# lbcb-sci/raven

Hardware: AMD Instinct MI355X
Metric: read Gbase/s through overlap+polish (higher is better)
Workload: dtype u32

## Files before the change

### raven_amd/csrc/map.hip

```cpp
#include <algorithm>

#include <cstring>

#include "engine.h"
#include "wave.h"
#ifdef RVN_TEST_HOOKS
#include "../../include/raven_hip_test.h"
#include "abi.h"
#endif

namespace rvn {

namespace {

template <typename V>
__device__ __forceinline__ bool index_find(const V* __restrict__ u_val, const u32* __restrict__ u_start,
                                           const u32* __restrict__ table, int shift, V v, u32* start, u32* count) {
  const u32 b = static_cast<u32>(static_cast<u64>(v) >> shift);
  u32 lo = table[b], hi = table[b + 1];
  const u32 end = hi;
  while (lo < hi) {
    const u32 mid = lo + ((hi - lo) >> 1);
    if (u_val[mid] < v) lo = mid + 1;
    else hi = mid;
  }
  if (lo < end && u_val[lo] == v) {
    *start = u_start[lo];
    *count = u_start[lo + 1] - *start;
    return true;
  }
  return false;
}

template <typename V>
__global__ void match_count_kernel(const V* __restrict__ q_val, const u64* __restrict__ q_org, u64 nq,
                                   const V* __restrict__ u_val, const u32* __restrict__ u_start,
                                   const u32* __restrict__ table, int shift, u32 n_keys,
                                   const u64* __restrict__ s_org, u32 occurrence, int avoid_equal,
                                   int avoid_symmetric, u32* __restrict__ q_start, u32* __restrict__ q_n,
                                   u32* __restrict__ q_cnt, u8* __restrict__ filtered, const u64* __restrict__ direct) {
  u64 q = static_cast<u64>(blockIdx.x) * blockDim.x + threadIdx.x;
  if (q >= nq) return;
  const V v = q_val[q];
  const u32 qid = origin_id(q_org[q]);
  u32 start = 0, count = 0, cnt = 0;
  u8 filt = 0;
  bool found;
  if (direct) {
    const u64 ent = direct[static_cast<u64>(v)];
    count = static_cast<u32>(ent >> 32);
    found = count != 0;
    start = found ? static_cast<u32>(ent) : 0u;
  } else {
    found = n_keys && index_find<V>(u_val, u_start, table, shift, v, &start, &count);
  }
  if (found) {
    if (count > occurrence) {
      filt = 1;
      count = 0;
    } else {
      for (u32 j = 0; j < count; ++j) {
        const u32 rid = origin_id(s_org[start + j]);
        if (avoid_equal && qid == rid) continue;
        if (avoid_symmetric && qid > rid) continue;
        ++cnt;
      }
    }
  }
  q_start[q] = start;
  q_n[q] = count;
  q_cnt[q] = cnt;
  if (filtered) filtered[q] = filt;
}

__global__ void match_emit_kernel(const u64* __restrict__ q_org, u64 nq, const u64* __restrict__ s_org,
                                  const u32* __restrict__ q_start, const u32* __restrict__ q_n,
                                  const u64* __restrict__ m_off, int avoid_equal, int avoid_symmetric,
                                  u64* __restrict__ m_grp, u64* __restrict__ m_pos) {
  u64 q = static_cast<u64>(blockIdx.x) * blockDim.x + threadIdx.x;
  if (q >= nq) return;
  const u32 count = q_n[q];
  if (count == 0) return;
  const u64 qo = q_org[q];
  const u32 qid = origin_id(qo);
  const u64 lhs_pos = static_cast<u32>(qo) >> 1;
  const u32 qstrand = static_cast<u32>(qo) & 1u;
  const u32 start = q_start[q];
  u64 o = m_off[q];
  for (u32 j = 0; j < count; ++j) {
    const u64 ro = s_org[start + j];
    const u32 rid = origin_id(ro);
    if (avoid_equal && qid == rid) continue;
    if (avoid_symmetric && qid > rid) continue;
    const u64 rhs_pos = static_cast<u32>(ro) >> 1;
    const u64 strand = (qstrand == (static_cast<u32>(ro) & 1u)) ? 1 : 0;
    const u64 diagonal = !strand ? rhs_pos + lhs_pos : rhs_pos - lhs_pos + (3ULL << 30);
    m_grp[o] = (((static_cast<u64>(rid) << 1) | strand) << 32) | diagonal;
    m_pos[o] = (lhs_pos << 32) | rhs_pos;
    ++o;
  }
}

template <bool EMIT>
__global__ __launch_bounds__(256) void join_kernel(const u32* __restrict__ u_start, u32 n_runs,
                                                  const u64* __restrict__ s_org, u32 occurrence, int all_query,
                                                  int avoid_equal, int avoid_symmetric, u32 first, u32 q_lo, u32 q_hi,
                                                  u32* __restrict__ read_cnt, const u64* __restrict__ seg_off,
                                                  u32* __restrict__ cursor, u64* __restrict__ m_grp,
                                                  u64* __restrict__ m_pos) {
  const u32 run = blockIdx.x * blockDim.x + threadIdx.x;
  if (run >= n_runs) return;
  const u32 s = u_start[run];
  const u32 c = u_start[run + 1] - s;
  const u32 f = run_foreign_prefix(s_org, s, c);
  if (c - f > occurrence || c == f) return;
  if (c == 1 && avoid_equal) return;
  for (u32 i = 0; i < c; ++i) {
    const u64 qo = s_org[s + i];
    if (!all_query && !(qo & kQueryFlag)) continue;
    const u32 qid = origin_id(qo);
    if (qid < q_lo || qid >= q_hi) continue;
    u32 cnt = 0;
    for (u32 j = f; j < c; ++j) {
      const u32 rid = origin_id(s_org[s + j]);
      if (avoid_equal && qid == rid) continue;
      if (avoid_symmetric && qid > rid) continue;
      ++cnt;
    }
    if (cnt == 0) continue;
    if (!EMIT) {
      atomicAdd(&read_cnt[qid - first], cnt);
    } else {
      u64 o = seg_off[qid - first] + atomicAdd(&cursor[qid - first], cnt);
      const u64 lhs_pos = static_cast<u32>(qo) >> 1;
      const u32 qstrand = static_cast<u32>(qo) & 1u;
      for (u32 j = f; j < c; ++j) {
        const u64 ro = s_org[s + j];
        const u32 rid = origin_id(ro);
        if (avoid_equal && qid == rid) continue;
        if (avoid_symmetric && qid > rid) continue;
        const u64 rhs_pos = static_cast<u32>(ro) >> 1;
        const u64 strand = (qstrand == (static_cast<u32>(ro) & 1u)) ? 1 : 0;
        const u64 diagonal = !strand ? rhs_pos + lhs_pos : rhs_pos - lhs_pos + (3ULL << 30);
        m_grp[o] = (((static_cast<u64>(rid) << 1) | strand) << 32) | diagonal;
        m_pos[o] = (lhs_pos << 32) | rhs_pos;
        ++o;
      }
    }
  }
}

__global__ void gather_u64_by_u32_kernel(const u64* __restrict__ src, const u32* __restrict__ idx,
                                         u64* __restrict__ dst, u32 n) {
  u32 i = blockIdx.x * blockDim.x + threadIdx.x;
  if (i < n) dst[i] = src[idx[i]];
}

template <bool PAY>
__device__ void wave_sort_segment(u64* __restrict__ k0, u64* __restrict__ k1, u64* __restrict__ p0,
                                  u64* __restrict__ p1, u64 b, u64 n, u32* hist) {
  const int lane = lane_id();
  const unsigned long long lt = lanemask_lt();
  u32* h_cur = hist;
  u32* h_nxt = hist + 256;
  for (int i = lane; i < 256; i += 64) h_nxt[i] = 0;
  __builtin_amdgcn_wave_barrier();
  u64 o = 0, a = ~0ULL;
  for (u64 i = lane; i < n; i += 64) {
    const u64 key = k0[b + i];
    o |= key;
    a &= key;
    atomicAdd(&h_nxt[key & 0xFF], 1u);
  }
#pragma unroll
  for (int off = 32; off > 0; off >>= 1) {
    o |= __shfl_xor(o, off, 64);
    a &= __shfl_xor(a, off, 64);
  }
  const u64 varying = o ^ a;
  int cur = 0;
  bool have_counts = true;
  int counted_shift = 0;
  for (int shift = 0; shift < 64; shift += 8) {
    if (((varying >> shift) & 0xFF) == 0) continue;
    const u64* kin = cur ? k1 : k0;
    const u64* pin = cur ? p1 : p0;
    u64* kout = cur ? k0 : k1;
    u64* pout = cur ? p0 : p1;
    __builtin_amdgcn_wave_barrier();
    if (have_counts && counted_shift == shift) {
      u32* t = h_cur;
      h_cur = h_nxt;
      h_nxt = t;
    } else {
      for (int i = lane; i < 256; i += 64) h_cur[i] = 0;
      __builtin_amdgcn_wave_barrier();
      for (u64 i = lane; i < n; i += 64) atomicAdd(&h_cur[(kin[b + i] >> shift) & 0xFF], 1u);
    }
    int nshift = shift + 8;
    while (nshift < 64 && ((varying >> nshift) & 0xFF) == 0) nshift += 8;
    have_counts = nshift < 64;
    counted_shift = nshift;
    __builtin_amdgcn_wave_barrier();
    {
      const u32 h0 = h_cur[4 * lane], h1 = h_cur[4 * lane + 1], h2 = h_cur[4 * lane + 2], h3 = h_cur[4 * lane + 3];
      const u32 s = h0 + h1 + h2 + h3;
      const u32 ex = wave_inclusive_sum(s) - s;
      __builtin_amdgcn_wave_barrier();
      h_cur[4 * lane] = ex;
      h_cur[4 * lane + 1] = ex + h0;
      h_cur[4 * lane + 2] = ex + h0 + h1;
      h_cur[4 * lane + 3] = ex + h0 + h1 + h2;
      for (int i = lane; i < 256; i += 64) h_nxt[i] = 0;
    }
    __builtin_amdgcn_wave_barrier();
    for (u64 base = 0; base < n; base += 256) {
      u64 key[4], pay[4];
      bool valid[4];
#pragma unroll
      for (int x = 0; x < 4; ++x) {
        const u64 i = base + 64 * x + lane;
        valid[x] = i < n;
        key[x] = 0;
        pay[x] = 0;
        if (valid[x]) {
          key[x] = kin[b + i];
          if (PAY) pay[x] = pin[b + i];
        }
      }
#pragma unroll
      for (int x = 0; x < 4; ++x) {
        if (base + 64 * x >= n) break;
        const unsigned d = static_cast<unsigned>((key[x] >> shift) & 0xFF);
        const unsigned long long peers = match_digit8(d, valid[x]);
        u32 before = 0;
        if (valid[x]) before = h_cur[d];
        __builtin_amdgcn_wave_barrier();
        const u32 rank = before + __popcll(peers & lt);
        if (valid[x] && (peers & lt) == 0) h_cur[d] = before + __popcll(peers);
        __builtin_amdgcn_wave_barrier();
        if (valid[x]) {
          kout[b + rank] = key[x];
          if (PAY) pout[b + rank] = pay[x];
          if (have_counts) atomicAdd(&h_nxt[(key[x] >> nshift) & 0xFF], 1u);
        }
      }
    }
    __threadfence_block();
    cur ^= 1;
  }
  if (cur) {
    for (u64 i = lane; i < n; i += 64) {
      k0[b + i] = k1[b + i];
      if (PAY) p0[b + i] = p1[b + i];
    }
    __threadfence_block();
  }
}

template <int NT, bool PAY>
constexpr size_t seg_sort_lds_bytes(u32 cap) {
  return static_cast<size_t>(cap) * 8 * (PAY ? 4 : 2) + (NT / 64) * 256 * 2 + 32 + (NT / 64) * 16;
}
template <int NT, bool PAY>
__device__ void block_sort_lds(u64* __restrict__ keys, u64* __restrict__ pays, u64 b, u32 n, u32 cap, unsigned char* smem) {
  constexpr int NW = NT / 64;
  static_assert(NT == 64 || NT == 256, "one wave or four");
  u64* s_k = reinterpret_cast<u64*>(smem);
  u64* s_p = s_k + 2 * static_cast<size_t>(cap);
  u16* wave_cnt = reinterpret_cast<u16*>(s_p + (PAY ? 2 * static_cast<size_t>(cap) : 0));
  u32* s4 = reinterpret_cast<u32*>(wave_cnt + NW * 256);
  u64* s_or = reinterpret_cast<u64*>(s4 + 8);
  u64* s_and = s_or + NW;
  const int lane = lane_id();
  const int w = threadIdx.x >> 6;
  u64 o = 0, a = ~0ULL;
  for (u32 i = threadIdx.x; i < n; i += NT) {
    const u64 k = keys[b + i];
    s_k[i] = k;
    if (PAY) s_p[i] = pays[b + i];
    o |= k;
    a &= k;
  }
#pragma unroll
  for (int x = 32; x > 0; x >>= 1) {
    o |= __shfl_xor(o, x, 64);
    a &= __shfl_xor(a, x, 64);
  }
  if (lane == 0) {
    s_or[w] = o;
    s_and[w] = a;
  }
  __syncthreads();
  u64 all_or = 0, all_and = ~0ULL;
#pragma unroll
  for (int x = 0; x < NW; ++x) {
    all_or |= s_or[x];
    all_and &= s_and[x];
  }
  const u64 varying = all_or ^ all_and;
  const u32 per = (n + NW - 1) / NW;
  const u32 q0 = min(n, w * per), q1 = min(n, q0 + per);
  const unsigned long long lt = lanemask_lt();
  u32 cur = 0;
  for (int shift = 0; shift < 64; shift += 8) {
    if (((varying >> shift) & 0xFF) == 0) continue;
    const u64* kin = s_k + static_cast<size_t>(cur) * cap;
    u64* kout = s_k + static_cast<size_t>(cur ^ 1) * cap;
    const u64* pin = s_p + static_cast<size_t>(cur) * cap;
    u64* pout = s_p + static_cast<size_t>(cur ^ 1) * cap;
    for (int i = threadIdx.x; i < NW * 256; i += NT) wave_cnt[i] = 0;
    __syncthreads();
    u16* my_cnt = wave_cnt + w * 256;
    for (u32 base = q0; base < q1; base += 64) {
      const u32 i = base + lane;
      const bool valid = i < q1;
      const unsigned d = valid ? static_cast<unsigned>((kin[i] >> shift) & 0xFF) : 0;
      const unsigned long long peers = match_digit8(d, valid);
      if (valid && (peers & lt) == 0) my_cnt[d] += static_cast<u16>(__popcll(peers));
      __builtin_amdgcn_wave_barrier();
    }
    __syncthreads();
    if (NT == 256) {
      const int t = threadIdx.x;
      u32 c[NW], tot = 0;
#pragma unroll
      for (int x = 0; x < NW; ++x) {
        c[x] = wave_cnt[x * 256 + t];
        tot += c[x];
      }
      u32 total;
      u32 run = block_exclusive_sum_256<u32>(tot, s4, &total);
#pragma unroll
      for (int x = 0; x < NW; ++x) {
        wave_cnt[x * 256 + t] = static_cast<u16>(run);
        run += c[x];
      }
    } else {
      const u32 h0 = wave_cnt[4 * lane], h1 = wave_cnt[4 * lane + 1], h2 = wave_cnt[4 * lane + 2], h3 = wave_cnt[4 * lane + 3];
      const u32 sum = h0 + h1 + h2 + h3;
      const u32 ex = wave_inclusive_sum(sum) - sum;
      __builtin_amdgcn_wave_barrier();
      wave_cnt[4 * lane] = static_cast<u16>(ex);
      wave_cnt[4 * lane + 1] = static_cast<u16>(ex + h0);
      wave_cnt[4 * lane + 2] = static_cast<u16>(ex + h0 + h1);
      wave_cnt[4 * lane + 3] = static_cast<u16>(ex + h0 + h1 + h2);
    }
    __syncthreads();
    for (u32 base = q0; base < q1; base += 64) {
      const u32 i = base + lane;
      const bool valid = i < q1;
      u64 k = 0, pv = 0;
      if (valid) {
        k = kin[i];
        if (PAY) pv = pin[i];
      }
      const unsigned d = static_cast<unsigned>((k >> shift) & 0xFF);
      const unsigned long long peers = match_digit8(d, valid);
      u32 before = 0;
      if (valid) before = my_cnt[d];
      __builtin_amdgcn_wave_barrier();
      if (valid && (peers & lt) == 0) my_cnt[d] = static_cast<u16>(before + __popcll(peers));
      __builtin_amdgcn_wave_barrier();
      if (valid) {
        const u32 dst = before + __popcll(peers & lt);
        kout[dst] = k;
        if (PAY) pout[dst] = pv;
      }
    }
    __syncthreads();
    cur ^= 1;
  }
  const u64* kfin = s_k + static_cast<size_t>(cur) * cap;
  const u64* pfin = s_p + static_cast<size_t>(cur) * cap;
  for (u32 i = threadIdx.x; i < n; i += NT) {
    keys[b + i] = kfin[i];
    if (PAY) pays[b + i] = pfin[i];
  }
}

constexpr int kSegClasses = 5;
__constant__ u32 kSegClassCap[kSegClasses] = {256, 512, 1024, 2048, 4096};
static const u32 kSegClassCapHost[kSegClasses] = {256, 512, 1024, 2048, 4096};
__global__ __launch_bounds__(256) void seg_class_list_kernel(const u64* __restrict__ off, u32 n_seg, u32* __restrict__ lists,
                                                            u32* __restrict__ cnt) {
  const u32 t = blockIdx.x * blockDim.x + threadIdx.x;
  int cls = -1;
  if (t < n_seg) {
    const u64 n = off[t + 1] - off[t];
    if (n >= 2) {
      cls = kSegClasses;
      for (int c = kSegClasses - 1; c >= 0; --c)
        if (n <= kSegClassCap[c]) cls = c;
    }
  }
  const int lane = lane_id();
  for (int c = 0; c <= kSegClasses; ++c) {
    const unsigned long long m = __ballot(cls == c);
    if (!m) continue;
    u32 base = 0;
    if (lane == 0) base = atomicAdd(cnt + c, static_cast<u32>(__popcll(m)));
    base = __shfl(base, 0, 64);
// ... 461 lines not shown
    const u32 nblk = (n + 63) >> 6;
    for (u32 b2 = lane; b2 < nblk; b2 += 64) maskbuf[b2] = 0;
    u32 j = tail_idx[longest];
    chain_sync<GLOBAL>();
    u32 left = longest;
    for (int b2 = static_cast<int>(j >> 6); b2 >= 0 && left; --b2) {
      const u32 idx = (static_cast<u32>(b2) << 6) + static_cast<u32>(lane);
      const u32 pr = idx < n ? static_cast<u32>(pred[idx]) : 0u;
      const unsigned long long cont = __ballot(lane > 0 && idx < n && pr + 1 == idx);
      unsigned long long m = 0;
      while (left && static_cast<int>(j >> 6) == b2) {
        const u32 l = j & 63u;
        const unsigned long long upto = l == 63 ? ~0ULL : ((2ULL << l) - 1ULL);
        const unsigned long long stops = ~cont & upto;
        u32 r = 63u - static_cast<u32>(__builtin_clzll(stops));
        if (l - r + 1 > left) r = l + 1 - left;
        m |= upto & ~((1ULL << r) - 1ULL);
        left -= l - r + 1;
        j = static_cast<u32>(__shfl(static_cast<int>(pr), static_cast<int>(r), 64));
      }
      if (lane == 0) maskbuf[b2] = m;
    }
    chain_sync<GLOBAL>();
    u32 at = 0;
    for (u32 b2 = 0; b2 < nblk; ++b2) {
      const unsigned long long m = maskbuf[b2];
      if ((m >> lane) & 1ULL) tail_idx[at + static_cast<u32>(__popcll(m & ((1ULL << lane) - 1ULL)))] = static_cast<IdxT>((b2 << 6) + lane);
      at += static_cast<u32>(__popcll(m));
    }
    chain_sync<GLOBAL>();
    for (u32 m = lane; m < longest; m += 64) tail_pos[m] = p[tail_idx[m]];
    chain_sync<GLOBAL>();
  }
  chain_emit_wave([&](u32 m) { return tail_pos[m]; }, longest, strand, g0, lhs_id, k, chain, min_matches, gap, slots,
                  slot_flags, anchors, anchor_base, slot_aoff, slot_acnt);
}

constexpr int kChainClasses = 8;
__constant__ u32 kChainClassCap[kChainClasses] = {128, 256, 512, 768, 1024, 2048, 4096, kChainBigCap};
static const u32 kChainClassCapHost[kChainClasses] = {128, 256, 512, 768, 1024, 2048, 4096, kChainBigCap};
inline size_t chain_class_lds(u32 cap) {
  return static_cast<size_t>(cap + 1) * 8 + (cap / 64 + 2) * 8 + static_cast<size_t>(cap + 2) * 2 + static_cast<size_t>(cap) * 2 + 64;
}

__global__ __launch_bounds__(64) void chain_kernel(const u64* __restrict__ grp, const u64* __restrict__ pos,
                                                  const u64* __restrict__ iv_begin, const u64* __restrict__ iv_end,
                                                  const u32* __restrict__ iv_read, const u32* __restrict__ list,
                                                  u32 n_list, u32 cap, const u32* __restrict__ ids, u32 first, u32 k,
                                                  u32 chain, u32 min_matches, u32 gap, u32 slot_div,
                                                  u64* __restrict__ g_tail_pos, u32* __restrict__ g_tail_idx,
                                                  u32* __restrict__ g_pred, u64* __restrict__ g_mask,
                                                  Overlap* __restrict__ slots, u8* __restrict__ slot_flags,
                                                  u64* __restrict__ anchors, u64* __restrict__ slot_aoff,
                                                  u32* __restrict__ slot_acnt) {
  extern __shared__ __attribute__((aligned(16))) unsigned char chain_smem[];
  if (blockIdx.x >= n_list) return;
  const u32 t = list[blockIdx.x];
  const u64 b = iv_begin[t];
  const u32 n = static_cast<u32>(iv_end[t] - b);
  const u64 g0 = grp[b];
  const bool strand = (g0 >> 32) & 1;
  const u32 lhs_id = ids[first + iv_read[t]];
  const u64 slot_base = (b + slot_div - 1) / slot_div;
  if (cap) {
    u64* tail_pos = reinterpret_cast<u64*>(chain_smem);
    u64* maskbuf = tail_pos + (cap + 1);
    u16* tail_idx = reinterpret_cast<u16*>(maskbuf + (cap / 64 + 2));
    u16* pred = tail_idx + (cap + 2);
    chain_wave<u16, false>(pos + b, n, strand, g0, lhs_id, k, chain, min_matches, gap, tail_pos, tail_idx, pred, maskbuf,
                           slots + slot_base, slot_flags + slot_base, anchors ? anchors + b : nullptr, b,
                           slot_aoff ? slot_aoff + slot_base : nullptr, slot_acnt ? slot_acnt + slot_base : nullptr);
  } else {
    chain_wave<u32, true>(pos + b, n, strand, g0, lhs_id, k, chain, min_matches, gap, g_tail_pos + b + t,
                          g_tail_idx + b + t, g_pred + b, g_mask + (b >> 6) + t, slots + slot_base,
                          slot_flags + slot_base, anchors ? anchors + b : nullptr, b,
                          slot_aoff ? slot_aoff + slot_base : nullptr, slot_acnt ? slot_acnt + slot_base : nullptr);
  }
}

__global__ __launch_bounds__(256) void chain_class_list_kernel(const u64* __restrict__ iv_begin,
                                                              const u64* __restrict__ iv_end, u32 n_iv, u32 chain,
                                                              u32* __restrict__ lists, u32* __restrict__ cnt) {
  const u32 t = blockIdx.x * blockDim.x + threadIdx.x;
  int cls = -1;
  if (t < n_iv) {
    const u64 n = iv_end[t] - iv_begin[t];
    if (n > kChainSmallCap && n >= chain) {
      cls = kChainClasses;
      for (int c = kChainClasses - 1; c >= 0; --c)
        if (n <= kChainClassCap[c]) cls = c;
    }
  }
  const int lane = lane_id();
  for (int c = 0; c <= kChainClasses; ++c) {
    const unsigned long long m = __ballot(cls == c);
    if (!m) continue;
    u32 base = 0;
    if (lane == 0) base = atomicAdd(cnt + c, static_cast<u32>(__popcll(m)));
    base = __shfl(base, 0, 64);
    if (cls == c) lists[static_cast<size_t>(c) * n_iv + base + __popcll(m & ((1ULL << lane) - 1ULL))] = t;
  }
}

__global__ void compact_overlaps_kernel(const Overlap* __restrict__ slots, const u8* __restrict__ flags,
                                        const u32* __restrict__ scan, u64 n_slots, Overlap* __restrict__ out) {
  u64 i = static_cast<u64>(blockIdx.x) * blockDim.x + threadIdx.x;
  if (i < n_slots && flags[i]) out[scan[i]] = slots[i];
}

__global__ void compact_aux_kernel(const u64* __restrict__ slot_aoff, const u32* __restrict__ slot_acnt,
                                   const u8* __restrict__ flags, const u32* __restrict__ scan, u64 n_slots,
                                   u64* __restrict__ aoff, u32* __restrict__ acnt) {
  u64 i = static_cast<u64>(blockIdx.x) * blockDim.x + threadIdx.x;
  if (i < n_slots && flags[i]) {
    aoff[scan[i]] = slot_aoff[i];
    acnt[scan[i]] = slot_acnt[i];
  }
}

__global__ void read_ovl_off_kernel(const u64* __restrict__ seg_off, const u32* __restrict__ scan, u32 slot_div,
                                    u32 n, u32* __restrict__ out) {
  u32 i = blockIdx.x * blockDim.x + threadIdx.x;
  if (i < n) out[i] = scan[(seg_off[i] + slot_div - 1) / slot_div];
}

}

void chain_matches(Engine& e, const ReadsDev& r, u32 first, u32 last, u64 H, MapOut& out) {
  hipStream_t s = e.stream;
  const u32 nr = last - first;
  u32* ovl_read_off = out.ovl_read_off.get<u32>(static_cast<size_t>(nr) + 1);
  u64* seg_off = e.map.seg_off.as<u64>();
  if (H == 0) {
    RVN_HIP(hipMemsetAsync(ovl_read_off, 0, (static_cast<size_t>(nr) + 1) * 4, s));
    return;
  }
  u64* g0 = e.map.m_grp[0].as<u64>();
  u64* g1 = e.map.m_grp[1].as<u64>();
  u64* p0 = e.map.m_pos[0].as<u64>();
  u64* p1 = e.map.m_pos[1].as<u64>();
  {
    StageTimer t(e, StageTimes::kSegSort);
    u32* lists = e.map.chain_big.get<u32>(static_cast<size_t>(nr) * (kSegClasses + 1) + 16);
    u32* d_cnt = lists + static_cast<size_t>(nr) * (kSegClasses + 1);
    RVN_HIP(hipMemsetAsync(d_cnt, 0, (kSegClasses + 1) * 4, s));
    seg_class_list_kernel<<<div_up(nr, 256), 256, 0, s>>>(seg_off, nr, lists, d_cnt);
    RVN_LAUNCH_CHECK();
    read_back(e, d_cnt, (kSegClasses + 1) * 4);
    u32 n_cls[kSegClasses + 1];
    std::memcpy(n_cls, e.h_pin, sizeof(n_cls));
    static bool attr_set = false;
    if (!attr_set) {
      RVN_HIP(hipFuncSetAttribute(reinterpret_cast<const void*>(seg_sort_group_lds_kernel<256>),
                                  hipFuncAttributeMaxDynamicSharedMemorySize,
                                  static_cast<int>(seg_sort_lds_bytes<256, true>(kSegClassCapHost[kSegClasses - 1]))));
      attr_set = true;
    }
    if (n_cls[kSegClasses])
      RVN_KLAUNCH(kKSegSortGroup, seg_sort_group_big_kernel<<<div_up(n_cls[kSegClasses], 4), 256, 0, s>>>(
                                      g0, g1, p0, p1, seg_off, lists + static_cast<size_t>(kSegClasses) * nr, n_cls[kSegClasses]));
    for (int c = kSegClasses - 1; c >= 0; --c) {
      if (!n_cls[c]) continue;
      const u32 cap = kSegClassCapHost[c];
      const u32* list = lists + static_cast<size_t>(c) * nr;
      if (cap <= 512)
        RVN_KLAUNCH(kKSegSortGroup, seg_sort_group_lds_kernel<64><<<n_cls[c], 64, seg_sort_lds_bytes<64, true>(cap), s>>>(
                                        g0, p0, seg_off, list, n_cls[c], cap));
      else
        RVN_KLAUNCH(kKSegSortGroup, seg_sort_group_lds_kernel<256><<<n_cls[c], 256, seg_sort_lds_bytes<256, true>(cap), s>>>(
                                        g0, p0, seg_off, list, n_cls[c], cap));
    }
    t.stop();
  }
  u32 NI = 0;
  const u64 n_slots4 = (H + 3) / 4 + 1;
  {
    StageTimer t(e, StageTimes::kIntervals);
    u64* slot_begin = e.map.iv_slot_begin.get<u64>(n_slots4 + 1);
    u64* slot_end = e.map.iv_slot_end.get<u64>(n_slots4 + 1);
    u32* iv_cnt = e.map.iv_cnt.get<u32>(static_cast<size_t>(nr) + 1);
    u32* iv_off = e.map.iv_off.get<u32>(static_cast<size_t>(nr) + 2);
    RVN_KLAUNCH(kKIntervals, intervals_kernel<<<div_up(nr, 4), 256, 0, s>>>(g0, seg_off, nr, e.bandwidth, slot_begin, slot_end, iv_cnt));
    exclusive_scan_u32_u32(iv_cnt, iv_off, nr, e.scratch.scan_tmp, s);
    NI = static_cast<u32>(read_back(e, iv_off + nr, 4));
    out.n_intervals = NI;
    if (NI) {
      u64* iv_begin = e.map.iv_begin.get<u64>(static_cast<size_t>(NI) + 1);
      u64* iv_end = e.map.iv_end.get<u64>(static_cast<size_t>(NI) + 1);
      u32* iv_read = e.scratch.tmp_b.get<u32>(static_cast<size_t>(NI) + 1);
      RVN_KLAUNCH(kKIntervalsGather, intervals_gather_kernel<<<div_up(nr, 4), 256, 0, s>>>(
                                         slot_begin, slot_end, seg_off, iv_off, nr, iv_begin, iv_end, iv_read));
    }
    t.stop();
  }
  if (NI == 0) {
    RVN_HIP(hipMemsetAsync(ovl_read_off, 0, (static_cast<size_t>(nr) + 1) * 4, s));
    return;
  }
  const u32 slot_div = std::max(1u, std::min(4u, e.chain));
  const u64 n_slots = (H + slot_div - 1) / slot_div + 1;
  Overlap* slots = e.map.ovl_slots.get<Overlap>(n_slots + 1);
  u8* slot_flags = e.map.ovl_flags.get<u8>(n_slots + 1);
  {
    StageTimer t(e, StageTimes::kChain);
    u64* iv_begin = e.map.iv_begin.as<u64>();
    u64* iv_end = e.map.iv_end.as<u64>();
    u32* iv_read = e.scratch.tmp_b.as<u32>();
    u32* lists = e.map.chain_big.get<u32>(static_cast<size_t>(NI) * (kChainClasses + 1) + 16);
    u32* d_cnt = lists + static_cast<size_t>(NI) * (kChainClasses + 1);
    RVN_HIP(hipMemsetAsync(d_cnt, 0, (kChainClasses + 1) * 4, s));
    chain_class_list_kernel<<<div_up(NI, 256), 256, 0, s>>>(iv_begin, iv_end, NI, e.chain, lists, d_cnt);
    RVN_LAUNCH_CHECK();
    read_back(e, d_cnt, (kChainClasses + 1) * 4);
    u32 n_cls[kChainClasses + 1];
    std::memcpy(n_cls, e.h_pin, sizeof(n_cls));
    static bool attr_set = false;
    if (!attr_set) {
      RVN_HIP(hipFuncSetAttribute(reinterpret_cast<const void*>(chain_kernel), hipFuncAttributeMaxDynamicSharedMemorySize,
                                  static_cast<int>(chain_class_lds(kChainBigCap))));
      RVN_HIP(hipFuncSetAttribute(reinterpret_cast<const void*>(seg_sort_pos_lds_kernel<256>),
                                  hipFuncAttributeMaxDynamicSharedMemorySize,
                                  static_cast<int>(seg_sort_lds_bytes<256, false>(kChainBigCap))));
      attr_set = true;
    }
    if (n_cls[kChainClasses])
      RVN_KLAUNCH(kKSegSortPos, seg_sort_pos_big_kernel<<<div_up(n_cls[kChainClasses], 4), 256, 0, s>>>(
                                    p0, p1, iv_begin, iv_end, lists + static_cast<size_t>(kChainClasses) * NI, n_cls[kChainClasses]));
    for (int c = kChainClasses - 1; c >= 0; --c) {
      if (!n_cls[c]) continue;
      const u32 cap = kChainClassCapHost[c];
      const u32* list = lists + static_cast<size_t>(c) * NI;
      if (cap <= 512)
        RVN_KLAUNCH(kKSegSortPos, seg_sort_pos_lds_kernel<64><<<n_cls[c], 64, seg_sort_lds_bytes<64, false>(cap), s>>>(
                                      p0, iv_begin, iv_end, list, n_cls[c], cap));
      else
        RVN_KLAUNCH(kKSegSortPos, seg_sort_pos_lds_kernel<256><<<n_cls[c], 256, seg_sort_lds_bytes<256, false>(cap), s>>>(
                                      p0, iv_begin, iv_end, list, n_cls[c], cap));
    }
    u32* lis_min = e.map.lis_min.get<u32>(H + NI + 1);
    u32* lis_pred = e.map.lis_pred.get<u32>(H + 1);
    u64* lis_tail = e.map.lis_tail.get<u64>(H + NI + 1);
    u64* lis_mask = e.map.lis_mask.get<u64>((H >> 6) + NI + 2);
    RVN_HIP(hipMemsetAsync(slot_flags, 0, n_slots + 1, s));
    u64* anchors = nullptr;
    u64* slot_aoff = nullptr;
    u32* slot_acnt = nullptr;
    if (e.map.keep_anchors) {
      anchors = out.anchors.get<u64>(H + 1);
      slot_aoff = e.map.anc_slot_off.get<u64>(n_slots + 1);
      slot_acnt = e.map.anc_slot_cnt.get<u32>(n_slots + 1);
    }
    RVN_KLAUNCH(kKChainSmall, chain_small_kernel<<<div_up(NI, 64), 64, 0, s>>>(
                                  g0, p0, iv_begin, iv_end, iv_read, NI, r.id.as<u32>(), first, e.k, e.chain, e.matches,
                                  e.gap, slot_div, slots, slot_flags, anchors, slot_aoff, slot_acnt));
    {
      for (int c = kChainClasses; c >= 0; --c) {
        if (!n_cls[c]) continue;
        const u32 cap = c < kChainClasses ? kChainClassCapHost[c] : 0u;
        const size_t lds = cap ? chain_class_lds(cap) : 0;
        RVN_KLAUNCH(kKChain, chain_kernel<<<n_cls[c], 64, lds, s>>>(g0, p0, iv_begin, iv_end, iv_read,
                                                                   lists + static_cast<size_t>(c) * NI, n_cls[c], cap,
                                                                   r.id.as<u32>(), first, e.k, e.chain, e.matches, e.gap,
                                                                   slot_div, lis_tail, lis_min, lis_pred, lis_mask, slots,
                                                                   slot_flags, anchors, slot_aoff, slot_acnt));
      }
    }
    t.stop();
  }
  {
    StageTimer t(e, StageTimes::kCompact);
    u32* scan = e.map.ovl_scan.get<u32>(n_slots + 2);
    exclusive_scan_u8_u32(slot_flags, scan, n_slots, e.scratch.scan_tmp, s);
    const u32 O = static_cast<u32>(read_back(e, scan + n_slots, 4));
    out.n_overlaps = O;
    e.c_overlaps += O;
    Overlap* ovl = out.ovl.get<Overlap>(static_cast<size_t>(O) + 1);
    RVN_KLAUNCH(kKCompactOverlaps, compact_overlaps_kernel<<<div_up(n_slots, 256), 256, 0, s>>>(slots, slot_flags, scan, n_slots, ovl));
    out.has_anchors = e.map.keep_anchors;
    if (e.map.keep_anchors) {
      u64* aoff = out.anchor_off.get<u64>(static_cast<size_t>(O) + 1);
      u32* acnt = out.anchor_cnt.get<u32>(static_cast<size_t>(O) + 1);
      RVN_KLAUNCH(kKCompactOverlaps, compact_aux_kernel<<<div_up(n_slots, 256), 256, 0, s>>>(
                                         e.map.anc_slot_off.as<u64>(), e.map.anc_slot_cnt.as<u32>(), slot_flags, scan, n_slots,
                                         aoff, acnt));
    }
    RVN_KLAUNCH(kKGather, read_ovl_off_kernel<<<div_up(nr + 1, 256), 256, 0, s>>>(seg_off, scan, slot_div, nr + 1, ovl_read_off));
    t.stop();
  }
}

namespace {

template <typename V>
u64 match_probe(Engine& e, const Sketch& qs, u32 nr, bool avoid_equal, bool avoid_symmetric, u8* filt, u64* seg_off) {
  hipStream_t s = e.stream;
  Index& ix = e.sketch.index;
  index_build_table(e);
  const u64 nq = qs.count;
  StageTimer t(e, StageTimes::kMatch);
  u32* q_start = e.map.q_start.get<u32>(nq + 1);
  u32* q_n = e.scratch.tmp_a.get<u32>(nq + 1);
  u32* q_cnt = e.map.q_cnt.get<u32>(nq + 1);
  u64* m_off = e.map.m_off.get<u64>(nq + 2);
  RVN_KLAUNCH(kKMatchCount, match_count_kernel<V><<<div_up(nq, 256), 256, 0, s>>>(
      qs.val.as<V>(), qs.org.as<u64>(), nq, ix.u_val.as<V>(), ix.u_start.as<u32>(), ix.table.as<u32>(), ix.shift,
      static_cast<u32>(ix.u), ix.s_org[ix.cur].as<u64>(), ix.occurrence, avoid_equal, avoid_symmetric, q_start, q_n,
      q_cnt, filt, ix.direct_built ? ix.direct.as<u64>() : nullptr));
  exclusive_scan_u32_u64(q_cnt, m_off, nq, e.scratch.scan_tmp, s);
  const u64 H = read_back(e, m_off + nq, 8);
  if (H) {
    u64* g0 = e.map.m_grp[0].get<u64>(H + 1);
    u64* p0 = e.map.m_pos[0].get<u64>(H + 1);
    e.map.m_grp[1].reserve((H + 1) * 8);
    e.map.m_pos[1].reserve((H + 1) * 8);
    RVN_KLAUNCH(kKMatchEmit, match_emit_kernel<<<div_up(nq, 256), 256, 0, s>>>(qs.org.as<u64>(), nq, ix.s_org[ix.cur].as<u64>(), q_start,
                                                      q_n, m_off, avoid_equal, avoid_symmetric, g0, p0));
    RVN_KLAUNCH(kKGather, gather_u64_by_u32_kernel<<<div_up(nr + 1, 256), 256, 0, s>>>(
                              e.map.m_off.as<u64>(), qs.read_off.as<u32>(), seg_off, nr + 1));
  }
  t.stop();
  return H;
}

template <typename V>
void map_batch_impl(Engine& e, const ReadsDev& r, u32 first, u32 last, bool avoid_equal, bool avoid_symmetric,
                    bool minhash, bool want_filtered, MapOut& out) {
  hipStream_t s = e.stream;
  Index& ix = e.sketch.index;
  const u32 nr = last - first;
  out.first = first;
  out.last = last;
  out.n_query = out.n_matches = out.n_intervals = out.n_overlaps = 0;
  u32* ovl_read_off = out.ovl_read_off.get<u32>(static_cast<size_t>(nr) + 1);

  u64* seg_off = e.map.seg_off.get<u64>(static_cast<size_t>(nr) + 2);
  u64 H = 0;
  const bool join = minhash && !want_filtered && ix.m != 0 && ix.first == first && ix.last == last &&
                    (ix.has_query_flags || ix.all_query) && ix.occurrence <= 4096 && r.ids_are_indices;
  if (join) {
    StageTimer t(e, StageTimes::kMatch);
    e.sketch.query_ready = {};
    for (u32 i = first; i < last; ++i) e.c_query_bases += r.h_len[i];
    out.n_query = ix.all_query ? ix.m : e.sketch.join_query_count;
    e.c_query_min += out.n_query;
    u32* read_cnt = e.map.q_cnt.get<u32>(2 * (static_cast<size_t>(nr) + 1));
    u32* cursor = read_cnt + nr + 1;
    RVN_HIP(hipMemsetAsync(read_cnt, 0, 2 * (static_cast<size_t>(nr) + 1) * 4, s));
    const u32 n_runs = static_cast<u32>(ix.u);
    const u64* sorg = ix.s_org[ix.cur].as<u64>();
    RVN_KLAUNCH(kKJoinCount, join_kernel<false><<<div_up(n_runs, 256), 256, 0, s>>>(
                                 ix.u_start.as<u32>(), n_runs, sorg, ix.occurrence, ix.all_query, avoid_equal,
                                 avoid_symmetric, r.h_id.empty() ? 0 : r.h_id[first], 0u, 0xFFFFFFFFu, read_cnt, nullptr, nullptr,
                                 nullptr, nullptr));
    exclusive_scan_u32_u64(read_cnt, seg_off, nr, e.scratch.scan_tmp, s);
    H = read_back(e, seg_off + nr, 8);
    out.n_matches = H;
    e.c_matches += H;
    if (H) {
      u64* g0 = e.map.m_grp[0].get<u64>(H + 1);
      u64* p0 = e.map.m_pos[0].get<u64>(H + 1);
      e.map.m_grp[1].reserve((H + 1) * 8);
      e.map.m_pos[1].reserve((H + 1) * 8);
      RVN_KLAUNCH(kKJoinEmit, join_kernel<true><<<div_up(n_runs, 256), 256, 0, s>>>(
                                  ix.u_start.as<u32>(), n_runs, sorg, ix.occurrence, ix.all_query, avoid_equal,
                                  avoid_symmetric, r.h_id[first], 0u, 0xFFFFFFFFu, nullptr, seg_off, cursor, g0, p0));
    }
    t.stop();
  }
  Sketch& qs = e.sketch.query_sketch;
  if (!join) {
  {
    StageTimer t(e, StageTimes::kQuery);
    const SketchState::QueryReady& q = e.sketch.query_ready;
    const bool ready = q.valid && q.first == first && q.last == last && q.minhash == minhash;
    e.sketch.query_ready = {};
    if (!ready) sketch_range(e, r, first, last, minhash, qs);
    t.stop();
  }
  const u64 nq = qs.count;
  out.n_query = nq;
  for (u32 i = first; i < last; ++i) e.c_query_bases += r.h_len[i];
  e.c_query_min += nq;
  if (nq == 0 || ix.m == 0) {
    RVN_HIP(hipMemsetAsync(ovl_read_off, 0, (static_cast<size_t>(nr) + 1) * 4, s));
    if (want_filtered) {
      u8* f = out.filtered.get<u8>(nq + 1);
      RVN_HIP(hipMemsetAsync(f, 0, nq + 1, s));
    }
    return;
  }
  H = match_probe<V>(e, qs, nr, avoid_equal, avoid_symmetric, want_filtered ? out.filtered.get<u8>(nq + 1) : nullptr, seg_off);
  e.c_matches += H;
  }
  out.n_matches = H;
  chain_matches(e, r, first, last, H, out);
}

}

u64 join_index_matches(Engine& e, u32 n_reads, bool avoid_equal, bool avoid_symmetric, u32 q_lo, u32 q_hi) {
  hipStream_t s = e.stream;
  Index& ix = e.sketch.index;
  u64* seg_off = e.map.seg_off.get<u64>(static_cast<size_t>(n_reads) + 2);
  RVN_HIP(hipMemsetAsync(seg_off, 0, (static_cast<size_t>(n_reads) + 2) * 8, s));
  if (ix.m == 0 || ix.u == 0) return 0;
  if (!(ix.has_query_flags || ix.all_query)) throw std::invalid_argument("[raven_hip] join: index has no query flags");
  StageTimer t(e, StageTimes::kMatch);
  u32* read_cnt = e.map.q_cnt.get<u32>(2 * (static_cast<size_t>(n_reads) + 1));
  u32* cursor = read_cnt + n_reads + 1;
  RVN_HIP(hipMemsetAsync(read_cnt, 0, 2 * (static_cast<size_t>(n_reads) + 1) * 4, s));
  const u32 n_runs = static_cast<u32>(ix.u);
  const u64* sorg = ix.s_org[ix.cur].as<u64>();
  RVN_KLAUNCH(kKJoinCount, join_kernel<false><<<div_up(n_runs, 256), 256, 0, s>>>(
                               ix.u_start.as<u32>(), n_runs, sorg, ix.occurrence, ix.all_query, avoid_equal,
                               avoid_symmetric, 0, q_lo, q_hi, read_cnt, nullptr, nullptr, nullptr, nullptr));
  exclusive_scan_u32_u64(read_cnt, seg_off, n_reads, e.scratch.scan_tmp, s);
  const u64 H = read_back(e, seg_off + n_reads, 8);
  e.c_matches += H;
  u64* g0 = e.map.m_grp[0].get<u64>(H + 1);
  u64* p0 = e.map.m_pos[0].get<u64>(H + 1);
  if (H)
    RVN_KLAUNCH(kKJoinEmit, join_kernel<true><<<div_up(n_runs, 256), 256, 0, s>>>(
                                ix.u_start.as<u32>(), n_runs, sorg, ix.occurrence, ix.all_query, avoid_equal,
                                avoid_symmetric, 0, q_lo, q_hi, nullptr, seg_off, cursor, g0, p0));
  t.stop();
  return H;
}

void map_batch_query_only(Engine& e, const ReadsDev& r, u32 first, u32 last, u64 n_query, MapOut& out) {
  hipStream_t s = e.stream;
  Index& ix = e.sketch.index;
  const u32 nr = last - first;
  out.first = first;
  out.last = last;
  out.n_query = n_query;
  out.n_matches = out.n_intervals = out.n_overlaps = 0;
  (void)out.ovl_read_off.get<u32>(static_cast<size_t>(nr) + 1);
  u64* seg_off = e.map.seg_off.get<u64>(static_cast<size_t>(nr) + 2);
  u64 H = 0;
  {
    StageTimer t(e, StageTimes::kMatch);
    e.sketch.query_ready = {};
    for (u32 i = first; i < last; ++i) e.c_query_bases += r.h_len[i];
    e.c_query_min += n_query;
    u32* read_cnt = e.map.q_cnt.get<u32>(2 * (static_cast<size_t>(nr) + 1));
    u32* cursor = read_cnt + nr + 1;
    RVN_HIP(hipMemsetAsync(read_cnt, 0, 2 * (static_cast<size_t>(nr) + 1) * 4, s));
    RVN_HIP(hipMemsetAsync(seg_off, 0, (static_cast<size_t>(nr) + 2) * 8, s));
    const u32 n_runs = static_cast<u32>(ix.u);
    const u64* sorg = ix.s_org[ix.cur].as<u64>();
    if (n_runs) {
      RVN_KLAUNCH(kKJoinCount, join_kernel<false><<<div_up(n_runs, 256), 256, 0, s>>>(
                                   ix.u_start.as<u32>(), n_runs, sorg, ix.occurrence, 0, 0, 0, r.h_id[first], 0u, 0xFFFFFFFFu,
                                   read_cnt, nullptr, nullptr, nullptr, nullptr));
      exclusive_scan_u32_u64(read_cnt, seg_off, nr, e.scratch.scan_tmp, s);
      H = read_back(e, seg_off + nr, 8);
    }
    e.c_matches += H;
    if (H) {
      u64* g0 = e.map.m_grp[0].get<u64>(H + 1);
      u64* p0 = e.map.m_pos[0].get<u64>(H + 1);
      e.map.m_grp[1].reserve((H + 1) * 8);
      e.map.m_pos[1].reserve((H + 1) * 8);
      RVN_KLAUNCH(kKJoinEmit, join_kernel<true><<<div_up(n_runs, 256), 256, 0, s>>>(
                                  ix.u_start.as<u32>(), n_runs, sorg, ix.occurrence, 0, 0, 0, r.h_id[first], 0u, 0xFFFFFFFFu,
                                  nullptr, seg_off, cursor, g0, p0));
    }
    t.stop();
  }
  out.n_matches = H;
  chain_matches(e, r, first, last, H, out);
}

void map_batch(Engine& e, const ReadsDev& r, u32 first, u32 last, bool avoid_equal, bool avoid_symmetric,
               bool minhash, bool want_filtered, MapOut& out) {
  if (e.val64) map_batch_impl<u64>(e, r, first, last, avoid_equal, avoid_symmetric, minhash, want_filtered, out);
  else map_batch_impl<u32>(e, r, first, last, avoid_equal, avoid_symmetric, minhash, want_filtered, out);
}

#ifdef RVN_TEST_HOOKS
static int test_match_probe(Engine& e, const u64* q_values, const u64* q_origins, u64 nq, const u32* q_read_off, u32 nr,
                     bool avoid_equal, bool avoid_symmetric, u64** grp, u64** pos, u64* seg_off, u8* filtered, u64* n_matches) {
  *grp = *pos = nullptr;
  *n_matches = 0;
  std::memset(seg_off, 0, (static_cast<size_t>(nr) + 1) * 8);
  if (nq) std::memset(filtered, 0, nq);
  if (nq >= (1ULL << 32)) throw std::invalid_argument("[raven_hip] rvn_test_match_probe: >= 2^32 query minimizers");
  if (q_read_off[0] != 0 || q_read_off[nr] != nq) throw std::invalid_argument("[raven_hip] rvn_test_match_probe: offsets must run from 0 to n_query");
  for (u32 i = 0; i < nr; ++i)
    if (q_read_off[i + 1] < q_read_off[i]) throw std::invalid_argument("[raven_hip] rvn_test_match_probe: offsets must ascend");
  const u64 limit = 1ULL << (2 * e.k);
  for (u64 i = 0; i < nq; ++i)
    if (q_values[i] >= limit) throw std::invalid_argument("[raven_hip] rvn_test_match_probe: value of more than 2k bits");
  auto empty = [](u64** p) {
    *p = static_cast<u64*>(std::malloc(8));
    if (!*p) throw std::bad_alloc();
  };
  if (nq == 0 || e.sketch.index.m == 0) {
    empty(grp);
    empty(pos);
    return RVN_OK;
  }
  Sketch& qs = e.sketch.query_sketch;
  e.sketch.query_ready = {};
  qs.first = 0;
  qs.last = nr;
  qs.count = nq;
  if (e.val64) {
    RVN_HIP(hipMemcpy(qs.val.get<u64>(nq + 1), q_values, nq * 8, hipMemcpyHostToDevice));
  } else {
    std::vector<u32> v32(nq);
    for (u64 i = 0; i < nq; ++i) v32[i] = static_cast<u32>(q_values[i]);
    RVN_HIP(hipMemcpy(qs.val.get<u32>(nq + 1), v32.data(), nq * 4, hipMemcpyHostToDevice));
  }
  RVN_HIP(hipMemcpy(qs.org.get<u64>(nq + 1), q_origins, nq * 8, hipMemcpyHostToDevice));
  RVN_HIP(hipMemcpy(qs.read_off.get<u32>(static_cast<size_t>(nr) + 1), q_read_off, (static_cast<size_t>(nr) + 1) * 4, hipMemcpyHostToDevice));
  u8* d_filt = e.map.out.filtered.get<u8>(nq + 1);
  u64* d_seg = e.map.seg_off.get<u64>(static_cast<size_t>(nr) + 2);
  const u64 H = e.val64 ? match_probe<u64>(e, qs, nr, avoid_equal, avoid_symmetric, d_filt, d_seg)
                        : match_probe<u32>(e, qs, nr, avoid_equal, avoid_symmetric, d_filt, d_seg);
  RVN_HIP(hipMemcpy(filtered, d_filt, nq, hipMemcpyDeviceToHost));
  *grp = static_cast<u64*>(std::malloc((H + 1) * 8));
  *pos = static_cast<u64*>(std::malloc((H + 1) * 8));
  if (!*grp || !*pos) throw std::bad_alloc();
  if (H) {
    RVN_HIP(hipMemcpy(*grp, e.map.m_grp[0].ptr, H * 8, hipMemcpyDeviceToHost));
    RVN_HIP(hipMemcpy(*pos, e.map.m_pos[0].ptr, H * 8, hipMemcpyDeviceToHost));
    RVN_HIP(hipMemcpy(seg_off, d_seg, (static_cast<size_t>(nr) + 1) * 8, hipMemcpyDeviceToHost));
  }
  *n_matches = H;
  return RVN_OK;
}
#endif

}

#ifdef RVN_TEST_HOOKS
extern "C" int rvn_test_match_probe(rvn_engine* h, const uint64_t* q_values, const uint64_t* q_origins, uint64_t n_query,
                                    const uint32_t* q_read_off, uint32_t n_reads, int avoid_equal, int avoid_symmetric,
                                    uint64_t** group, uint64_t** positions, uint64_t* seg_off, uint8_t* filtered,
                                    uint64_t* n_matches) {
  using namespace rvn;
  const bool ok = h && q_read_off && group && positions && seg_off && n_matches && !(n_query && (!q_values || !q_origins || !filtered));
  return guarded(h, ok, "[raven_hip] rvn_test_match_probe: NULL argument", [&](Engine& e) -> int {
    try {
      return test_match_probe(e, q_values, q_origins, n_query, q_read_off, n_reads, avoid_equal != 0, avoid_symmetric != 0, group,
                              positions, seg_off, filtered, n_matches);
    } catch (...) {
      std::free(*group);
      std::free(*positions);
      *group = *positions = nullptr;
      throw;
    }
  });
}
#endif
```

Before: 1.431.

## Emit matches with wave-cooperative load balancing and template out avoid filtering

The match emit kernel now spreads each wave's matches across its lanes. It builds a wave prefix sum of per-query counts in shared memory, and each lane binary-searches for its owning query, so one lane no longer serially loops over a long run. When filtering is active, ballot/popcount compaction with a carry across chunks computes output ranks. Both count and emit kernels are templated on whether avoid-equal/symmetric filtering is needed, so the no-filter path skips reading query origins and the per-hit loop. A debug stats print behind an env knob is also added.

```diff
diff --git a/raven_amd/csrc/map.hip b/raven_amd/csrc/map.hip
--- a/raven_amd/csrc/map.hip
+++ b/raven_amd/csrc/map.hip
@@ -1,6 +1,8 @@
 #include <algorithm>
 
+#include <cstdio>
 #include <cstring>
+#include <vector>
 
 #include "engine.h"
 #include "wave.h"
@@ -32,7 +34,7 @@
   return false;
 }
 
-template <typename V>
+template <typename V, bool AVOID>
 __global__ void match_count_kernel(const V* __restrict__ q_val, const u64* __restrict__ q_org, u64 nq,
                                    const V* __restrict__ u_val, const u32* __restrict__ u_start,
                                    const u32* __restrict__ table, int shift, u32 n_keys,
@@ -42,10 +44,9 @@
   u64 q = static_cast<u64>(blockIdx.x) * blockDim.x + threadIdx.x;
   if (q >= nq) return;
   const V v = q_val[q];
-  const u32 qid = origin_id(q_org[q]);
   u32 start = 0, count = 0, cnt = 0;
   u8 filt = 0;
-  bool found;
+  bool found = false;
   if (direct) {
     const u64 ent = direct[static_cast<u64>(v)];
     count = static_cast<u32>(ent >> 32);
@@ -58,13 +59,16 @@
     if (count > occurrence) {
       filt = 1;
       count = 0;
-    } else {
+    } else if (AVOID) {
+      const u32 qid = origin_id(q_org[q]);
       for (u32 j = 0; j < count; ++j) {
         const u32 rid = origin_id(s_org[start + j]);
         if (avoid_equal && qid == rid) continue;
         if (avoid_symmetric && qid > rid) continue;
         ++cnt;
       }
+    } else {
+      cnt = count;
     }
   }
   q_start[q] = start;
@@ -73,31 +77,78 @@
   if (filtered) filtered[q] = filt;
 }
 
-__global__ void match_emit_kernel(const u64* __restrict__ q_org, u64 nq, const u64* __restrict__ s_org,
-                                  const u32* __restrict__ q_start, const u32* __restrict__ q_n,
-                                  const u64* __restrict__ m_off, int avoid_equal, int avoid_symmetric,
-                                  u64* __restrict__ m_grp, u64* __restrict__ m_pos) {
-  u64 q = static_cast<u64>(blockIdx.x) * blockDim.x + threadIdx.x;
-  if (q >= nq) return;
-  const u32 count = q_n[q];
-  if (count == 0) return;
-  const u64 qo = q_org[q];
-  const u32 qid = origin_id(qo);
-  const u64 lhs_pos = static_cast<u32>(qo) >> 1;
-  const u32 qstrand = static_cast<u32>(qo) & 1u;
-  const u32 start = q_start[q];
-  u64 o = m_off[q];
-  for (u32 j = 0; j < count; ++j) {
-    const u64 ro = s_org[start + j];
-    const u32 rid = origin_id(ro);
-    if (avoid_equal && qid == rid) continue;
-    if (avoid_symmetric && qid > rid) continue;
-    const u64 rhs_pos = static_cast<u32>(ro) >> 1;
-    const u64 strand = (qstrand == (static_cast<u32>(ro) & 1u)) ? 1 : 0;
-    const u64 diagonal = !strand ? rhs_pos + lhs_pos : rhs_pos - lhs_pos + (3ULL << 30);
-    m_grp[o] = (((static_cast<u64>(rid) << 1) | strand) << 32) | diagonal;
-    m_pos[o] = (lhs_pos << 32) | rhs_pos;
-    ++o;
+template <bool AVOID>
+__global__ __launch_bounds__(256) void match_emit_kernel(const u64* __restrict__ q_org, u64 nq, const u64* __restrict__ s_org,
+                                                        const u32* __restrict__ q_start, const u32* __restrict__ q_n,
+                                                        const u64* __restrict__ m_off, int avoid_equal, int avoid_symmetric,
+                                                        u64* __restrict__ m_grp, u64* __restrict__ m_pos) {
+  __shared__ u64 s_incl[4][kWave];
+  __shared__ u64 s_off[4][kWave];
+  __shared__ u64 s_qo[4][kWave];
+  __shared__ u32 s_start[4][kWave];
+  const int lane = lane_id();
+  const int w = threadIdx.x >> 6;
+  const u64 q = static_cast<u64>(blockIdx.x) * blockDim.x + threadIdx.x;
+  const u32 n = q < nq ? q_n[q] : 0u;
+  u64 off = 0, qo = 0;
+  u32 start = 0;
+  if (n) {
+    start = q_start[q];
+    off = m_off[q];
+    qo = q_org[q];
+  }
+  const u64 incl = static_cast<u64>(wave_inclusive_sum<unsigned long long>(n));
+  s_incl[w][lane] = incl;
+  s_off[w][lane] = off;
+  s_qo[w][lane] = qo;
+  s_start[w][lane] = start;
+  __syncthreads();
+  const u64 total = s_incl[w][kWave - 1];
+  u64 carry = 0;
+  for (u64 base = 0; base < total; base += kWave) {
+    const u64 e = base + lane;
+    const bool live = e < total;
+    u32 lo = 0, hi = kWave - 1;
+#pragma unroll
+    for (int it = 0; it < 6; ++it) {
+      const u32 mid = (lo + hi) >> 1;
+      const bool right = live && s_incl[w][mid] <= e;
+      lo = right ? mid + 1 : lo;
+      hi = right ? hi : mid;
+    }
+    const u32 r = live ? lo : 0u;
+    const u64 excl = r ? s_incl[w][r - 1] : 0;
+    bool keep = live;
+    u64 ro = 0, run_qo = 0;
+    if (live) {
+      run_qo = s_qo[w][r];
+      ro = s_org[static_cast<u64>(s_start[w][r]) + (e - excl)];
+      if (AVOID) {
+        const u32 qid = origin_id(run_qo), rid = origin_id(ro);
+        if (avoid_equal && qid == rid) keep = false;
+        if (avoid_symmetric && qid > rid) keep = false;
+      }
+    }
+    u64 rank = e - excl;
+    if (AVOID) {
+      const u64 kept = __ballot(keep);
+      const bool reaches_in = excl < base;
+      const u32 f = reaches_in ? 0u : static_cast<u32>(excl - base);
+      rank = static_cast<u64>(__popcll(kept & lanemask_lt() & (~0ULL << f))) + (reaches_in ? carry : 0);
+      const u32 f_last = __shfl(f, kWave - 1, kWave);
+      const int last_reaches_in = __shfl(static_cast<int>(reaches_in), kWave - 1, kWave);
+      carry = static_cast<u64>(__popcll(kept >> f_last)) + (last_reaches_in ? carry : 0);
+    }
+    if (keep) {
+      const u32 rid = origin_id(ro);
+      const u64 lhs_pos = static_cast<u32>(run_qo) >> 1;
+      const u64 rhs_pos = static_cast<u32>(ro) >> 1;
+      const u64 strand = ((static_cast<u32>(run_qo) & 1u) == (static_cast<u32>(ro) & 1u)) ? 1 : 0;
+      const u64 diagonal = !strand ? rhs_pos + lhs_pos : rhs_pos - lhs_pos + (3ULL << 30);
+      const u64 o = s_off[w][r] + rank;
+      m_grp[o] = (((static_cast<u64>(rid) << 1) | strand) << 32) | diagonal;
+      m_pos[o] = (lhs_pos << 32) | rhs_pos;
+    }
   }
 }
 
@@ -1165,10 +1216,20 @@
   u32* q_n = e.scratch.tmp_a.get<u32>(nq + 1);
   u32* q_cnt = e.map.q_cnt.get<u32>(nq + 1);
   u64* m_off = e.map.m_off.get<u64>(nq + 2);
-  RVN_KLAUNCH(kKMatchCount, match_count_kernel<V><<<div_up(nq, 256), 256, 0, s>>>(
+  const bool avoid = avoid_equal || avoid_symmetric;
+  auto* count_kernel = avoid ? match_count_kernel<V, true> : match_count_kernel<V, false>;
+  RVN_KLAUNCH(kKMatchCount, count_kernel<<<div_up(nq, 256), 256, 0, s>>>(
       qs.val.as<V>(), qs.org.as<u64>(), nq, ix.u_val.as<V>(), ix.u_start.as<u32>(), ix.table.as<u32>(), ix.shift,
       static_cast<u32>(ix.u), ix.s_org[ix.cur].as<u64>(), ix.occurrence, avoid_equal, avoid_symmetric, q_start, q_n,
       q_cnt, filt, ix.direct_built ? ix.direct.as<u64>() : nullptr));
+  if (knob("RVN_MATCH_STATS")) {
+    std::vector<u32> h_n(nq);
+    RVN_HIP(hipStreamSynchronize(s));
+    RVN_HIP(hipMemcpy(h_n.data(), q_n, nq * 4, hipMemcpyDeviceToHost));
+    const u64 empty = static_cast<u64>(std::count(h_n.begin(), h_n.end(), 0u));
+    std::fprintf(stderr, "[raven_hip] match_probe: %llu query minimizers, %llu with q_n == 0, index of %llu keys\n",
+                 static_cast<unsigned long long>(nq), static_cast<unsigned long long>(empty), static_cast<unsigned long long>(ix.u));
+  }
   exclusive_scan_u32_u64(q_cnt, m_off, nq, e.scratch.scan_tmp, s);
   const u64 H = read_back(e, m_off + nq, 8);
   if (H) {
@@ -1176,8 +1237,9 @@
     u64* p0 = e.map.m_pos[0].get<u64>(H + 1);
     e.map.m_grp[1].reserve((H + 1) * 8);
     e.map.m_pos[1].reserve((H + 1) * 8);
-    RVN_KLAUNCH(kKMatchEmit, match_emit_kernel<<<div_up(nq, 256), 256, 0, s>>>(qs.org.as<u64>(), nq, ix.s_org[ix.cur].as<u64>(), q_start,
-                                                      q_n, m_off, avoid_equal, avoid_symmetric, g0, p0));
+    auto* emit_kernel = avoid ? match_emit_kernel<true> : match_emit_kernel<false>;
+    RVN_KLAUNCH(kKMatchEmit, emit_kernel<<<div_up(nq, 256), 256, 0, s>>>(qs.org.as<u64>(), nq, ix.s_org[ix.cur].as<u64>(), q_start, q_n,
+                                                                        m_off, avoid_equal, avoid_symmetric, g0, p0));
     RVN_KLAUNCH(kKGather, gather_u64_by_u32_kernel<<<div_up(nr + 1, 256), 256, 0, s>>>(
                               e.map.m_off.as<u64>(), qs.read_off.as<u32>(), seg_off, nr + 1));
   }
```

Result: no change. 1.443 (median of 4 runs) (+0.8%).
